# kyshu11027/financial-chatbot-llm

Hardware: AMD Instinct MI355X
Metric: chat turns/sec + p50 TTFT, Llama-3-8B RAG agent at 1/2/4/8 MI355X (higher is better)
Workload: dtype bf16

## Files before the change

financial_chatbot_llm_amd/csrc/kernels/gemm_prefill.hip:

```cpp
#include "common.h"
#include "kv_layout.h"

#include <type_traits>

namespace {

constexpr int TN = 256;
constexpr int TM = 256;
constexpr int BK = 64;
constexpr int HALF = 128 * 128;
constexpr int BUF = 4 * HALF;
constexpr int GM = 4;
enum { H_W0 = 0, H_X0 = 1, H_X1 = 2, H_W1 = 3 };
enum { EPI_BF16 = 0, EPI_SILU = 1, EPI_SLAB = 2, EPI_RESID = 3, EPI_ROPE = 4, EPI_BIAS = 5, EPI_BIAS_GELU = 6,
       EPI_MOE_SILU = 7, EPI_MOE_ROUTE = 8, EPI_SAMPLE = 9, EPI_MOE_SILU_MX = 10, EPI_MOE_ROUTE_MX = 11,
       EPI_LOGPROB = 12, EPI_SAMPLE_LP = 13 };

struct MoeArgs {
  const int* offsets;
  const int* rows;
  const float* xs;
  const float* ws;
  const float* route_w;
  int E;
  unsigned* mxs;
  int nkt;
};

struct SampleArgs {
  const float* temps;
  const unsigned long long* seeds;
  float* pv;
  int* pi;
  int voff, vvalid;
};

struct LogprobArgs {
  const int* targets;
  float* pm;
  float* ps;
  float* pt;
  int* pa;
  int voff, vvalid;
};

struct TailArgs {
  int dpn, L, s;
  float* part;
  int* cnt;
  int gm = 0;
};

struct RopeArgs {
  const int* positions;
  const float* cos_sin;
  const int* slots;
  bf16* q_out;
  bf16* k_cache;
  bf16* v_cache;
  int Hq, Hkv;
  float qscale = 1.f;
};

template <bool FP8>
__device__ __forceinline__ int swz(int r) { return FP8 ? ((r >> 1) & 5) : ((r >> 1) & 7); }

union Frag {
  uint4 u;
  bf16x8 v;
};
typedef int i32x8 __attribute__((ext_vector_type(8)));
union FragPair {
  Frag f[2];
  i32x8 v;
};

__device__ __forceinline__ uint4 pair16(bf16x4 lo, bf16x4 hi) {
  union {
    bf16x4 v;
    uint2 u;
  } a, b;
  a.v = lo;
  b.v = hi;
  const auto x = __builtin_amdgcn_permlane16_swap(a.u.x, b.u.x, false, false);
  const auto y = __builtin_amdgcn_permlane16_swap(a.u.y, b.u.y, false, false);
  return make_uint4(x[0], y[0], x[1], y[1]);
}

template <int N>
__device__ __forceinline__ void wait_vm() {
  asm volatile("s_waitcnt vmcnt(%0)" ::"n"(N) : "memory");
}
__device__ __forceinline__ void wait_lgkm0() { asm volatile("s_waitcnt lgkmcnt(0)" ::: "memory"); }
__device__ __forceinline__ void bar() { __builtin_amdgcn_s_barrier(); }

__device__ __forceinline__ void read_w(const char* __restrict__ h, FragPair (&a)[4], int wa, int rowoff,
                                       const int (&choff)[2]) {
#pragma unroll
  for (int f = 0; f < 4; ++f)
#pragma unroll
    for (int kk = 0; kk < 2; ++kk)
      a[f].f[kk].u = *reinterpret_cast<const uint4*>(h + (wa * 64 + f * 16) * 128 + rowoff + choff[kk]);
}

__device__ __forceinline__ void read_w_tiled(const char* __restrict__ h, FragPair (&a)[4], int wa, int lane) {
#pragma unroll
  for (int f = 0; f < 4; ++f)
#pragma unroll
    for (int kk = 0; kk < 2; ++kk)
      a[f].f[kk].u = *reinterpret_cast<const uint4*>(h + ((wa * 4 + f) * 2 + kk) * 1024 + lane * 16);
}

__device__ __forceinline__ void read_x(const char* __restrict__ h, FragPair (&b)[2], int wb, int rowoff,
                                       const int (&choff)[2]) {
#pragma unroll
  for (int t = 0; t < 2; ++t)
#pragma unroll
    for (int kk = 0; kk < 2; ++kk)
      b[t].f[kk].u = *reinterpret_cast<const uint4*>(h + (wb * 32 + t * 16) * 128 + rowoff + choff[kk]);
}

template <int F0, int T0, bool FP8, bool MXI = false>
__device__ __forceinline__ void mma(f32x4 (&acc)[8][4], const FragPair (&a)[4], const FragPair (&b)[2],
                                    unsigned sc = 0) {
  __builtin_amdgcn_sched_barrier(0);
  __builtin_amdgcn_s_setprio(1);
  if constexpr (FP8 && MXI) {
#pragma unroll
    for (int f = 0; f < 4; ++f) {
      acc[F0 + f][T0] = __builtin_amdgcn_mfma_scale_f32_16x16x128_f8f6f4(a[f].v, b[0].v, acc[F0 + f][T0], 0, 0, 0,
                                                                         127, T0, (int)sc);
      acc[F0 + f][T0 + 1] = __builtin_amdgcn_mfma_scale_f32_16x16x128_f8f6f4(a[f].v, b[1].v, acc[F0 + f][T0 + 1], 0, 0,
                                                                             0, 127, T0 + 1, (int)sc);
    }
#pragma unroll
    for (int f = 0; f < 4; ++f)
#pragma unroll
      for (int t = 0; t < 2; ++t) asm volatile("" : "+v"(acc[F0 + f][T0 + t]));
  } else if constexpr (FP8) {
#pragma unroll
    for (int f = 0; f < 4; ++f)
#pragma unroll
      for (int t = 0; t < 2; ++t)
        acc[F0 + f][T0 + t] = __builtin_amdgcn_mfma_scale_f32_16x16x128_f8f6f4(
            a[f].v, b[t].v, acc[F0 + f][T0 + t], 0, 0, 0, 127, 0, 127);
#pragma unroll
    for (int f = 0; f < 4; ++f)
#pragma unroll
      for (int t = 0; t < 2; ++t) asm volatile("" : "+v"(acc[F0 + f][T0 + t]));
  } else {
#pragma unroll
    for (int kk = 0; kk < 2; ++kk)
#pragma unroll
      for (int f = 0; f < 4; ++f)
#pragma unroll
        for (int t = 0; t < 2; ++t)
          acc[F0 + f][T0 + t] =
              __builtin_amdgcn_mfma_f32_16x16x32_bf16(a[f].f[kk].v, b[t].f[kk].v, acc[F0 + f][T0 + t], 0, 0, 0);
  }
  __builtin_amdgcn_s_setprio(0);
  __builtin_amdgcn_sched_barrier(0);
}

template <int EPI, int ABL = 0, int BAL = 1, bool FP8 = false, bool WT = false>
__global__ void __launch_bounds__(512) gemm_prefill_kernel(const void* __restrict__ Xv, int ldx,
                                                           const void* __restrict__ Wv, int K,
                                                           void* __restrict__ Y, int ldy,
                                                           const bf16* __restrict__ R, int ldr,
                                                           int M, int N, int S, RopeArgs ra, MoeArgs ma,
                                                           SampleArgs sa, TailArgs ta, LogprobArgs la) {
  static_assert(!(WT && FP8), "fragment-tiled W: bf16 only");
  constexpr int ESZ = FP8 ? 1 : 2;
  constexpr int BKE = 128 / ESZ;
  constexpr bool MXI = EPI == EPI_MOE_ROUTE_MX;
  constexpr bool MXO = EPI == EPI_MOE_SILU_MX;
  static_assert(!(MXI || MXO) || (FP8 && BAL), "MX hand-off: fp8 tiles on the balanced schedule");
  constexpr int XL0 = MXI ? 3 : 2;
  const char* __restrict__ X = static_cast<const char*>(Xv);
  const char* __restrict__ W = static_cast<const char*>(Wv);
  __shared__ __attribute__((aligned(1024))) char smem[2 * BUF + (MXI ? 2048 : 0)];
  const int lane = threadIdx.x & 63;
  const int w = __builtin_amdgcn_readfirstlane(threadIdx.x >> 6);
  const int wa = w >> 2, wb = w & 3;
  const int g = lane >> 4, col = lane & 15;

  const int Mt = (M + TM - 1) / TM + (FP8 ? ma.E : 0), Nt = N / TN, tiles = Mt * Nt;
  const bool tail = !FP8 && EPI != EPI_SAMPLE_LP && ta.s > 1 && (int)blockIdx.x >= ta.dpn;
  int s = 0, tile, tu = 0, tj = 0;
  if (tail) {
    const int u = blockIdx.x - ta.dpn;
    tu = u % ta.L;
    tj = u / ta.L;
    tile = ta.dpn + tu;
  } else {
    const int nwg = ta.s > 1 ? ta.dpn : tiles * S;
    int id = blockIdx.x;
    const int xcd = id & 7, q = nwg >> 3, r = nwg & 7;
    id = (xcd < r ? xcd * (q + 1) : r * (q + 1) + (xcd - r) * q) + (id >> 3);
    s = id / tiles;
    tile = id - s * tiles;
  }
  const int GMr = ta.gm > 0 ? ta.gm : GM;
  const int grp = tile / (GMr * Nt), first = grp * GMr, gm = min(Mt - first, GMr);
  const int within = tile - grp * GMr * Nt;
  const int tm = first + within % gm, tn = within / gm;
  int m0 = tm * TM, mend = M, e = 0;
  const int n0 = tn * TN;
  if constexpr (FP8) {
    int rem = tm;
    for (e = 0; e < ma.E; ++e) {
      const int lo = ma.offsets[e], hi = ma.offsets[e + 1], nte = (hi - lo + TM - 1) / TM;
      if (rem < nte) {
        m0 = lo + rem * TM;
        mend = hi;
        break;
      }
      rem -= nte;
    }
    if (e == ma.E) return;
    W += (long)e * N * K;
  }
  int k0, nt;
  if (tail) {
    const int ntot = K / BKE, kb = tj * ntot / ta.s, ke = (tj + 1) * ntot / ta.s;
    k0 = kb * BKE;
    nt = ke - kb;
  } else {
    const int kc = K / S;
    k0 = s * kc;
    nt = kc / BKE;
  }
  PENNY_DASSERT(N % TN == 0 && nt >= 1 && tm < Mt && tn < Nt);

  const char* src[4][2];
  unsigned soff[4][2];
#pragma unroll
  for (int h = 0; h < 4; ++h)
#pragma unroll
    for (int i = 0; i < 2; ++i) {
      const int lr = 16 * w + 8 * i + (lane >> 3);
      const int c = (lane & 7) ^ swz<FP8>(lr);
      if (h == H_W0 || h == H_W1) {
        const int n = n0 + (lr >> 6) * 128 + (h == H_W1 ? 64 : 0) + (lr & 63);
        if constexpr (FP8) soff[h][i] = (unsigned)(((long)n * K + k0) + 16 * c);
        else if constexpr (WT) {
          const int G = n0 / 16 + (w >> 2) * 8 + (w & 3) + (h == H_W1 ? 4 : 0);
          src[h][i] = W + (((long)G * (K / 32) + k0 / 32 + i) * 64 + lane) * 16;
        } else src[h][i] = W + ((long)n * K + k0) * ESZ + 16 * c;
      } else {
        int m = min(m0 + (lr >> 5) * 64 + (h == H_X1 ? 32 : 0) + (lr & 31), mend - 1);
        if (FP8 && ma.rows) m = ma.rows[m];
        if constexpr (FP8) soff[h][i] = (unsigned)(((long)m * ldx + k0) + 16 * c);
        else src[h][i] = X + ((long)m * ldx + k0) * ESZ + 16 * c;
      }
    }
  const unsigned lds0 = (unsigned)(uintptr_t)((__attribute__((address_space(3))) char*)smem);
  const char* mxbase = nullptr;
  if constexpr (MXI) mxbase = reinterpret_cast<const char*>(ma.mxs) + ((long)tm * ma.nkt + k0 / BKE) * 1024 + w * 128;
  auto stage = [&](int h, int t, unsigned buf) {
    if (ABL == 1 && t > 1) return;
#pragma unroll
    for (int i = 0; i < 2; ++i) {
      const unsigned dst = buf + h * HALF + (16 * w + 8 * i) * 128;
      unsigned keep;
      if constexpr (FP8) {
        const unsigned vo = soff[h][i] + (unsigned)t * 128;
        const char* base = (h == H_W0 || h == H_W1) ? W : X;
        asm volatile("s_mov_b32 %0, m0\n\ts_mov_b32 m0, %2\n\ts_nop 0\n\tglobal_load_lds_dwordx4 %1, %3\n\ts_mov_b32 m0, %0"
                     : "=&s"(keep)
                     : "v"(vo), "s"(dst), "s"(base)
                     : "memory");
      } else {
        const char* gp = src[h][i] + (long)t * ((WT && (h == H_W0 || h == H_W1)) ? 2048 : 128);
        asm volatile("s_mov_b32 %0, m0\n\ts_mov_b32 m0, %2\n\ts_nop 0\n\tglobal_load_lds_dwordx4 %1, off\n\ts_mov_b32 m0, %0"
                     : "=&s"(keep)
                     : "v"(gp), "s"(dst)
                     : "memory");
      }
    }
    if constexpr (MXI) {
      if (h == H_X0) {
        const char* gp = mxbase + (long)t * 1024 + lane * 4;
        const unsigned dst = lds0 + 2 * BUF + (t & 1) * 1024 + w * 128;
        unsigned keep;
        if (lane < 32)
          asm volatile("s_mov_b32 %0, m0\n\ts_mov_b32 m0, %2\n\ts_nop 0\n\tglobal_load_lds_dword %1, off\n\ts_mov_b32 m0, %0"
                       : "=&s"(keep)
                       : "v"(gp), "s"(dst)
                       : "memory");
      }
    }
  };
  auto read_sc = [&](int t) -> unsigned {
    if constexpr (MXI)
      return *reinterpret_cast<const unsigned*>(smem + 2 * BUF + (t & 1) * 1024 + wb * 256 + col * 16 + g * 4);
    else
      return 0u;
  };

  const int rowoff = col * 128;
  const int choff[2] = {((FP8 ? 2 * g : g) ^ swz<FP8>(col)) << 4, ((FP8 ? 2 * g + 1 : 4 + g) ^ swz<FP8>(col)) << 4};

  f32x4 acc[8][4];
#pragma unroll
  for (int f = 0; f < 8; ++f)
#pragma unroll
// ... 15 lines not shown
    wait_vm<0>();
  }
  bar();
  if (wa == 1) bar();

  auto phase = [&](auto F0c, auto T0c, const FragPair (&aa)[4], const FragPair (&bb)[2], unsigned sc = 0) {
    constexpr int F0 = decltype(F0c)::value, T0 = decltype(T0c)::value;
    bar();
    wait_lgkm0();
    mma<F0, T0, FP8, MXI>(acc, aa, bb, sc);
    bar();
  };
  using I0 = std::integral_constant<int, 0>;
  using I2 = std::integral_constant<int, 2>;
  using I4 = std::integral_constant<int, 4>;

  if constexpr (BAL) {
    FragPair c0[2];
    unsigned sc = 0;
    auto tile = [&](int t, FragPair (&bc)[2], FragPair (&bn)[2]) {
      const char* cur = smem + (t & 1) * BUF;
      const char* nx = smem + ((t + 1) & 1) * BUF;
      const unsigned lcur = lds0 + (t & 1) * BUF, lnxt = lds0 + ((t + 1) & 1) * BUF;
      const bool more1 = t + 1 < nt, more2 = t + 2 < nt;
      if (ABL != 2 || t == 0) READ_W(cur + H_W0 * HALF);
      sc = read_sc(t);
      if (more1) stage(H_W1, t + 1, lnxt);
      phase(I0{}, I0{}, a, bc, sc);
      if (ABL != 2 || t == 0) read_x(cur + H_X1 * HALF, b1, wb, rowoff, choff);
      if (more2) stage(H_W0, t + 2, lcur);
      phase(I0{}, I2{}, a, b1, sc);
      if (ABL != 2 || t == 0) READ_W(cur + H_W1 * HALF);
      if (more2) {
        stage(H_X0, t + 2, lcur);
        if (ABL != 3) wait_vm<6 + XL0>();
      } else {
        wait_vm<0>();
      }
      phase(I4{}, I2{}, a, b1, sc);
      if (more1 && (ABL != 2 || t == 0)) read_x(nx + H_X0 * HALF, bn, wb, rowoff, choff);
      if (more2) {
        stage(H_X1, t + 2, lcur);
        if (ABL != 3) wait_vm<4 + XL0>();
      } else {
        wait_vm<0>();
      }
      phase(I4{}, I0{}, a, bc, sc);
    };
    read_x(smem + H_X0 * HALF, b0, wb, rowoff, choff);
    int t = 0;
    for (; t + 1 < nt; t += 2) {
      tile(t, b0, c0);
      tile(t + 1, c0, b0);
    }
    if (t < nt) tile(t, b0, c0);
  } else {
    for (int t = 0; t < nt; ++t) {
      const char* cur = smem + (t & 1) * BUF;
      const unsigned lcur = lds0 + (t & 1) * BUF, lnxt = lds0 + ((t + 1) & 1) * BUF;
      const bool more1 = t + 1 < nt, more2 = t + 2 < nt;
      if (ABL != 2 || t == 0) {
        READ_W(cur + H_W0 * HALF);
        read_x(cur + H_X0 * HALF, b0, wb, rowoff, choff);
      }
      if (more1) stage(H_W1, t + 1, lnxt);
      phase(I0{}, I0{}, a, b0);
      if (ABL != 2 || t == 0) read_x(cur + H_X1 * HALF, b1, wb, rowoff, choff);
      if (more2) stage(H_W0, t + 2, lcur);
      phase(I0{}, I2{}, a, b1);
      if (ABL != 2 || t == 0) READ_W(cur + H_W1 * HALF);
      if (more2) stage(H_X0, t + 2, lcur);
      phase(I4{}, I2{}, a, b1);
      if (more2) {
        stage(H_X1, t + 2, lcur);
        if (ABL != 3) wait_vm<6>();
      } else {
        wait_vm<0>();
      }
      phase(I4{}, I0{}, a, b0);
    }
  }
  if (wa == 0) bar();

  if (!FP8 && tail) {
    float* mine = ta.part + ((long)tu * ta.s + tj) * (TM * TN);
#pragma unroll
    for (int f = 0; f < 8; ++f)
#pragma unroll
      for (int t = 0; t < 4; ++t)
        *reinterpret_cast<f32x4*>(mine + ((((w * 8 + f) * 4 + t) * 64 + lane) << 2)) = acc[f][t];
    wait_vm<0>();
    __syncthreads();
    int* flag = reinterpret_cast<int*>(smem);
    if (threadIdx.x == 0) {
      __builtin_amdgcn_fence(__ATOMIC_RELEASE, "agent");
      wait_vm<0>();
      const int old = __hip_atomic_fetch_add(&ta.cnt[tu], 1, __ATOMIC_RELAXED, __HIP_MEMORY_SCOPE_AGENT);
      const int last = old == ta.s - 1;
      if (last) {
        __builtin_amdgcn_fence(__ATOMIC_ACQUIRE, "agent");
        wait_vm<0>();
        __hip_atomic_store(&ta.cnt[tu], 0, __ATOMIC_RELAXED, __HIP_MEMORY_SCOPE_AGENT);
      }
      *reinterpret_cast<volatile int*>(flag) = last;
    }
    __syncthreads();
    if (!*reinterpret_cast<volatile int*>(flag)) return;
    const float* base = ta.part + (long)tu * ta.s * (TM * TN) + ((w * 32 * 64 + lane) << 2);
    for (int j = 0; j < ta.s; ++j) {
      const float* pj = base + (long)j * (TM * TN);
#pragma unroll
      for (int f = 0; f < 8; ++f)
#pragma unroll
        for (int t = 0; t < 4; ++t) {
          const f32x4 v = *reinterpret_cast<const f32x4*>(pj + ((f * 4 + t) * 64 << 2));
          acc[f][t] = j == 0 ? v : acc[f][t] + v;
        }
    }
  }

  const int lane_off = 8 * (g >> 1) + 16 * (g & 1);
  if constexpr (MXO) {
    const float* wsc = ma.ws + (long)e * N + n0 + wa * 128;
    unsigned char* yq = static_cast<unsigned char*>(Y);
    const int ocol = ((n0 + wa * 128) >> 1) + 4 * g;
    unsigned word[2] = {0u, 0u};
#pragma unroll
    for (int t = 0; t < 4; ++t) {
      const int m = m0 + wb * 64 + t * 16 + col;
      const bool valid = m < mend;
      const int mr = min(m, mend - 1);
      const float sx = ma.xs[ma.rows ? ma.rows[mr] : mr];
      float o[4][4];
#pragma unroll
      for (int q = 0; q < 4; ++q) {
        const f32x4 sg = *reinterpret_cast<const f32x4*>(wsc + 32 * q + 4 * g);
        const f32x4 su = *reinterpret_cast<const f32x4*>(wsc + 32 * q + 16 + 4 * g);
#pragma unroll
        for (int r = 0; r < 4; ++r) {
          const float gv = (float)(bf16)(acc[2 * q][t][r] * sx * sg[r]);
          const float uv = (float)(bf16)(acc[2 * q + 1][t][r] * sx * su[r]);
          o[q][r] = (float)(bf16)((float)(bf16)(gv / (1.f + __expf(-gv))) * uv);
        }
      }
#pragma unroll
      for (int bb = 0; bb < 2; ++bb) {
        float amax = 0.f;
#pragma unroll
        for (int q = bb; q < 4; q += 2)
#pragma unroll
          for (int r = 0; r < 4; ++r) amax = fmaxf(amax, fabsf(o[q][r]));
        amax = fmaxf(amax, __shfl_xor(amax, 16, 64));
        amax = fmaxf(amax, __shfl_xor(amax, 32, 64));
        const unsigned bits = __float_as_uint(amax * (1.f / 448.f));
        const int ex = (int)((bits >> 23) & 0xff);
        int X = ex == 0 ? -127 : ex - 127 + ((bits & 0x7fffff) != 0);
        X = max(-127, min(X, 126));
        word[bb] |= (unsigned)(X + 127) << (8 * t);
        const float inv = __uint_as_float((unsigned)(127 - X) << 23);
        if (valid) {
#pragma unroll
          for (int q = bb; q < 4; q += 2) {
            uint32_t pk = 0;
            pk = __builtin_amdgcn_cvt_pk_fp8_f32(o[q][0] * inv, o[q][1] * inv, pk, false);
            pk = __builtin_amdgcn_cvt_pk_fp8_f32(o[q][2] * inv, o[q][3] * inv, pk, true);
            *reinterpret_cast<uint32_t*>(yq + (long)m * ldy + ocol + 16 * q) = pk;
          }
        }
      }
    }
    if (g < 2)
      ma.mxs[((long)tm * ma.nkt + n0 / 256) * 256 + wb * 64 + col * 4 + wa + 2 * g] = g == 0 ? word[0] : word[1];
    return;
  }
#pragma unroll
  for (int t = 0; t < 4; ++t) {
    const int m = m0 + wb * 64 + t * 16 + col;
    if (m >= mend) continue;
    if constexpr (EPI == EPI_MOE_SILU || EPI == EPI_MOE_ROUTE || EPI == EPI_MOE_ROUTE_MX) {
      const float sx = MXI ? 1.f : ma.xs[ma.rows ? ma.rows[m] : m];
      const float* wsc = ma.ws + (long)e * N + n0 + wa * 128;
      if constexpr (EPI == EPI_MOE_SILU) {
        bf16x4 o[4];
#pragma unroll
        for (int q = 0; q < 4; ++q) {
          const f32x4 sg = *reinterpret_cast<const f32x4*>(wsc + 32 * q + 4 * g);
          const f32x4 su = *reinterpret_cast<const f32x4*>(wsc + 32 * q + 16 + 4 * g);
#pragma unroll
          for (int r = 0; r < 4; ++r) {
            const float gv = (float)(bf16)(acc[2 * q][t][r] * sx * sg[r]);
            const float uv = (float)(bf16)(acc[2 * q + 1][t][r] * sx * su[r]);
            o[q][r] = (bf16)((float)(bf16)(gv / (1.f + __expf(-gv))) * uv);
          }
        }
        bf16* y = static_cast<bf16*>(Y) + (long)m * ldy + ((n0 + wa * 128) >> 5) * 16 + lane_off;
#pragma unroll
        for (int q = 0; q < 4; q += 2) *reinterpret_cast<uint4*>(y + 16 * q) = pair16(o[q], o[q + 1]);
      } else {
        const float rw = sx * ma.route_w[m];
        bf16* y = static_cast<bf16*>(Y) + (long)m * ldy + n0 + wa * 128 + lane_off;
// ... 124 lines not shown
      const long blk = slot >= 0 ? slot / KV_BS : 0;
      const int off = slot >= 0 ? slot % KV_BS : 0;
      if (hd < ra.Hq + ra.Hkv) {
        const float* cs = ra.cos_sin + (long)ra.positions[m] * D;
        const float qs = hd < ra.Hq ? ra.qscale : 1.f;
#pragma unroll
        for (int f = 0; f < 4; ++f) {
          const int d = f * 16 + 4 * g;
          const f32x4 co = *reinterpret_cast<const f32x4*>(cs + d), si = *reinterpret_cast<const f32x4*>(cs + 64 + d);
          bf16x4 o1, o2;
#pragma unroll
          for (int r = 0; r < 4; ++r) {
            const float x1 = (float)(bf16)acc[f][t][r], x2 = (float)(bf16)acc[f + 4][t][r];
            o1[r] = (bf16)((x1 * co[r] - x2 * si[r]) * qs);
            o2[r] = (bf16)((x2 * co[r] + x1 * si[r]) * qs);
          }
          if (hd < ra.Hq) {
            bf16* q = ra.q_out + ((long)m * ra.Hq + hd) * D;
            *reinterpret_cast<bf16x4*>(q + d) = o1;
            *reinterpret_cast<bf16x4*>(q + 64 + d) = o2;
          } else {
            bf16* kb = ra.k_cache + (blk * ra.Hkv + (hd - ra.Hq)) * (long)(KV_BS * D);
            *reinterpret_cast<bf16x4*>(kb + k_index(off, d, D)) = o1;
            *reinterpret_cast<bf16x4*>(kb + k_index(off, 64 + d, D)) = o2;
          }
        }
      } else {
        bf16* vb = ra.v_cache + (blk * ra.Hkv + (hd - ra.Hq - ra.Hkv)) * (long)(KV_BS * D);
#pragma unroll
        for (int f = 0; f < 8; ++f)
#pragma unroll
          for (int r = 0; r < 4; ++r) vb[v_index(off, f * 16 + 4 * g + r, D)] = (bf16)acc[f][t][r];
      }
    } else if constexpr (EPI == EPI_SILU) {
      const int col0 = ((n0 + wa * 128) >> 5) * 16;
      bf16x4 o[4];
#pragma unroll
      for (int q = 0; q < 4; ++q)
#pragma unroll
        for (int r = 0; r < 4; ++r) {
          const float gt = (float)(bf16)acc[2 * q][t][r], up = (float)(bf16)acc[2 * q + 1][t][r];
          o[q][r] = (bf16)((float)(bf16)(gt / (1.f + __expf(-gt))) * up);
        }
      bf16* y = static_cast<bf16*>(Y) + (long)m * ldy + col0 + lane_off;
#pragma unroll
      for (int q = 0; q < 4; q += 2) *reinterpret_cast<uint4*>(y + 16 * q) = pair16(o[q], o[q + 1]);
    } else if constexpr (EPI == EPI_SLAB) {
      float* P = static_cast<float*>(Y) + (long)s * M * N + (long)m * N;
#pragma unroll
      for (int f = 0; f < 8; ++f) *reinterpret_cast<f32x4*>(P + n0 + wa * 128 + f * 16 + 4 * g) = acc[f][t];
    } else {
      bf16* y = static_cast<bf16*>(Y) + (long)m * ldy + n0 + wa * 128 + lane_off;
#pragma unroll
      for (int f = 0; f < 8; f += 2) {
        bf16x4 lo, hi;
        if constexpr (EPI == EPI_BIAS || EPI == EPI_BIAS_GELU) {
          const int n = n0 + wa * 128 + f * 16 + 4 * g;
          const bf16x4 b0 = *reinterpret_cast<const bf16x4*>(R + n), b1 = *reinterpret_cast<const bf16x4*>(R + n + 16);
#pragma unroll
          for (int r = 0; r < 4; ++r) {
            float u0 = (float)(bf16)(acc[f][t][r] + (float)b0[r]), u1 = (float)(bf16)(acc[f + 1][t][r] + (float)b1[r]);
            if constexpr (EPI == EPI_BIAS_GELU) {
              u0 = 0.5f * u0 * (1.f + erff(u0 * 0.70710678118654752f));
              u1 = 0.5f * u1 * (1.f + erff(u1 * 0.70710678118654752f));
            }
            lo[r] = (bf16)u0, hi[r] = (bf16)u1;
          }
        } else {
#pragma unroll
          for (int r = 0; r < 4; ++r) lo[r] = (bf16)acc[f][t][r], hi[r] = (bf16)acc[f + 1][t][r];
        }
        Pack8 v;
        v.u = pair16(lo, hi);
        if constexpr (EPI == EPI_RESID) {
          Pack8 rr;
          rr.u = *reinterpret_cast<const uint4*>(R + (long)m * ldr + n0 + wa * 128 + lane_off + 16 * f);
#pragma unroll
          for (int j = 0; j < 8; ++j) v.e[j] = (bf16)((float)v.e[j] + (float)rr.e[j]);
        }
        *reinterpret_cast<uint4*>(y + 16 * f) = v.u;
      }
    }
  }
}

}

#undef READ_W

static int g_group = 0;

template <int EPI, int ABL = 0, int BAL = 1, bool WT = false>
static void launch(dim3 grid, hipStream_t stream, const void* X, int ldx, const void* W, int K, void* Y, int ldy,
                   const void* R, int ldr, int M, int N, int S, const RopeArgs& ra, TailArgs ta = TailArgs{}) {
  ta.gm = g_group;
  hipLaunchKernelGGL((gemm_prefill_kernel<EPI, ABL, BAL, false, WT>), grid, dim3(512), 0, stream, X, ldx, W, K, Y,
                     ldy, (const bf16*)R, ldr, M, N, S, ra, MoeArgs{}, SampleArgs{}, ta, LogprobArgs{});
}

static dim3 grid_for(int M, int N, int S) { return dim3((unsigned)(((M + TM - 1) / TM) * (N / TN) * S)); }

static dim3 tail_plan(int M, int N, int K, int cus, float* ws, long ws_floats, int* cnt, int ncnt, TailArgs& ta) {
  ta = TailArgs{};
  const int T = ((M + TM - 1) / TM) * (N / TN);
  if (cus > 0 && ws && cnt) {
    const int L = T % cus, ntot = K / BK;
    int s = L ? cus / L : 0;
    s = min(s, ntot / 16);
    if (L && s >= 2 && L <= ncnt && (long)L * s * TM * TN <= ws_floats) {
      ta = TailArgs{T - L, L, s, ws, cnt};
      return dim3((unsigned)(T - L + L * s));
    }
  }
  return dim3((unsigned)T);
}

PENNY_API int penny_gemm_prefill_set_group(int gm) {
  if (gm < 0 || gm > 64) return (int)hipErrorInvalidValue;
  g_group = gm;
  return 0;
}

PENNY_API int penny_gemm_prefill(const void* X, int ldx, const void* W, int K, void* Y, int ldy, const void* R,
                                 int ldr, int M, int N, int S, int epi, float* tail_ws, long tail_ws_floats,
                                 int* tail_cnt, int tail_ncnt, int cus, hipStream_t stream) {
  if (M <= 0) return 0;
  if (N % TN || S < 1 || K % (BK * S) || ldx % 8 || epi < 0 || epi > 6 || epi == EPI_ROPE)
    return (int)hipErrorInvalidValue;
  if (epi != EPI_SLAB && (S != 1 || ldy % 8)) return (int)hipErrorInvalidValue;
  if (epi == EPI_RESID && (!R || ldr % 8)) return (int)hipErrorInvalidValue;
  if ((epi == EPI_BIAS || epi == EPI_BIAS_GELU) && !R) return (int)hipErrorInvalidValue;
  if ((long)((M + TM - 1) / TM) * (N / TN) * S > (1L << 30)) return (int)hipErrorInvalidValue;
  TailArgs ta{};
  const dim3 grid = S == 1 ? tail_plan(M, N, K, cus, tail_ws, tail_ws_floats, tail_cnt, tail_ncnt, ta)
                           : grid_for(M, N, S);
  const RopeArgs ra{};
  switch (epi) {
    case EPI_BF16: launch<EPI_BF16>(grid, stream, X, ldx, W, K, Y, ldy, R, ldr, M, N, S, ra, ta); break;
    case EPI_SILU: launch<EPI_SILU>(grid, stream, X, ldx, W, K, Y, ldy, R, ldr, M, N, S, ra, ta); break;
    case EPI_SLAB: launch<EPI_SLAB>(grid, stream, X, ldx, W, K, Y, ldy, R, ldr, M, N, S, ra); break;
    case EPI_BIAS: launch<EPI_BIAS>(grid, stream, X, ldx, W, K, Y, ldy, R, ldr, M, N, S, ra, ta); break;
    case EPI_BIAS_GELU: launch<EPI_BIAS_GELU>(grid, stream, X, ldx, W, K, Y, ldy, R, ldr, M, N, S, ra, ta); break;
    default: launch<EPI_RESID>(grid, stream, X, ldx, W, K, Y, ldy, R, ldr, M, N, S, ra, ta);
  }
  return (int)hipGetLastError();
}

PENNY_API int penny_gemm_prefill_wt(const void* X, int ldx, const void* Wt, int K, void* Y, int ldy, const void* R,
                                    int ldr, int M, int N, int S, int epi, float* tail_ws, long tail_ws_floats,
                                    int* tail_cnt, int tail_ncnt, int cus, hipStream_t stream) {
  if (M <= 0) return 0;
  if (N % TN || S < 1 || K % (BK * S) || ldx % 8 || (epi != EPI_BF16 && epi != EPI_SILU && epi != EPI_SLAB &&
                                                    epi != EPI_RESID))
    return (int)hipErrorInvalidValue;
  if (epi != EPI_SLAB && (S != 1 || ldy % 8)) return (int)hipErrorInvalidValue;
  if (epi == EPI_RESID && (!R || ldr % 8)) return (int)hipErrorInvalidValue;
  TailArgs ta{};
  const dim3 grid = S == 1 ? tail_plan(M, N, K, cus, tail_ws, tail_ws_floats, tail_cnt, tail_ncnt, ta)
                           : grid_for(M, N, S);
  const RopeArgs ra{};
  switch (epi) {
    case EPI_BF16: launch<EPI_BF16, 0, 1, true>(grid, stream, X, ldx, Wt, K, Y, ldy, R, ldr, M, N, S, ra, ta); break;
    case EPI_SILU: launch<EPI_SILU, 0, 1, true>(grid, stream, X, ldx, Wt, K, Y, ldy, R, ldr, M, N, S, ra, ta); break;
    case EPI_SLAB: launch<EPI_SLAB, 0, 1, true>(grid, stream, X, ldx, Wt, K, Y, ldy, R, ldr, M, N, S, ra); break;
    default: launch<EPI_RESID, 0, 1, true>(grid, stream, X, ldx, Wt, K, Y, ldy, R, ldr, M, N, S, ra, ta);
  }
  return (int)hipGetLastError();
}

PENNY_API int penny_gemm_prefill_qkv_rope(const void* X, int ldx, const void* W, int K, int M, const int* positions,
                                          const float* cos_sin, const int* slots, void* q_out, void* k_cache,
                                          void* v_cache, int Hq, int Hkv, float qscale, float* tail_ws,
                                          long tail_ws_floats,
                                          int* tail_cnt, int tail_ncnt, int cus, hipStream_t stream) {
  if (M <= 0) return 0;
  const int N = (Hq + 2 * Hkv) * 128;
  if (Hq <= 0 || Hkv <= 0 || N % TN || K % BK || ldx % 8 || !positions || !cos_sin || !slots || !q_out)
    return (int)hipErrorInvalidValue;
  const RopeArgs ra{positions, cos_sin, slots, (bf16*)q_out, (bf16*)k_cache, (bf16*)v_cache, Hq, Hkv, qscale};
  TailArgs ta{};
  const dim3 grid = tail_plan(M, N, K, cus, tail_ws, tail_ws_floats, tail_cnt, tail_ncnt, ta);
  launch<EPI_ROPE>(grid, stream, X, ldx, W, K, nullptr, 0, nullptr, 0, M, N, 1, ra, ta);
  return (int)hipGetLastError();
}

PENNY_API int penny_gemm_prefill_ablate(const void* X, int ldx, const void* W, int K, void* Y, int ldy, int M, int N,
                                        int ablate, hipStream_t stream) {
  if (M <= 0) return 0;
  if (N % TN || K % BK || ldx % 8 || ldy % 4) return (int)hipErrorInvalidValue;
  const RopeArgs ra{};
  if (ablate == 1) launch<EPI_BF16, 1>(grid_for(M, N, 1), stream, X, ldx, W, K, Y, ldy, nullptr, 0, M, N, 1, ra);
  else if (ablate == 10) launch<EPI_BF16, 0, 0>(grid_for(M, N, 1), stream, X, ldx, W, K, Y, ldy, nullptr, 0, M, N, 1, ra);
  else if (ablate == 3) launch<EPI_BF16, 3>(grid_for(M, N, 1), stream, X, ldx, W, K, Y, ldy, nullptr, 0, M, N, 1, ra);
  else if (ablate == 2) launch<EPI_BF16, 2>(grid_for(M, N, 1), stream, X, ldx, W, K, Y, ldy, nullptr, 0, M, N, 1, ra);
  else launch<EPI_BF16, 0>(grid_for(M, N, 1), stream, X, ldx, W, K, Y, ldy, nullptr, 0, M, N, 1, ra);
  return (int)hipGetLastError();
}

PENNY_API int penny_moe_gemm_prefill_fp8(const void* X, int ldx, const int* rows, const float* xs, const int* offsets,
                                         const void* W, const float* ws, const float* route_w, void* Y, int ldy,
                                         int P, int E, int N, int K, int epi, hipStream_t stream) {
  if (P <= 0) return 0;
  const bool plain = epi >= 16;
// ... 296 lines not shown
```

financial_chatbot_llm_amd/ops/_native.py:

```python
from __future__ import annotations

import ctypes
import os
import threading
from typing import Optional

import torch

_LOCK = threading.Lock()
_LIB: Optional[ctypes.CDLL] = None
_ERR: Optional[str] = None

c_int, c_long, c_float, c_void_p = ctypes.c_int, ctypes.c_long, ctypes.c_float, ctypes.c_void_p
P = c_void_p

_SIGS = {
    "penny_rmsnorm": [P, P, P, P, c_int, c_int, c_float, c_int, P],
    "penny_rmsnorm_slabs": [P, c_int, P, P, P, c_int, c_int, c_float, c_int, P],
    "penny_layernorm": [P, P, P, P, P, c_int, c_int, c_float, c_int, P],
    "penny_silu_mul": [P, P, c_int, c_int, c_int, P],
    "penny_skinny_gemm": [P, c_int, P, c_int, P, c_int, P, c_int, c_int, c_int, c_int, c_int, c_int, P],
    "penny_splitk_gemm": [P, c_int, P, c_int, P, c_int, c_int, c_int, c_int, c_int, P],
    "penny_splitk_reduce": [P, c_int, c_int, c_int, P, c_int, P, c_int, P],
    "penny_splitk_gemm_bf16": [P, c_int, P, c_int, P, c_int, c_int, c_int, c_int, c_int, P],
    "penny_lm_head_stream_sample": [P, c_int, P, c_int, c_int, c_int, c_int, c_int, P, P, P, P, P, c_int, c_int,
                                    c_int, P],
    "penny_lm_sample_final": [P, P, c_int, c_int, P, P, P],
    "penny_gateup_silu_gemm": [P, c_int, P, c_int, P, c_int, c_int, c_int, c_int, c_int, P],
    "penny_gemm_prefill": [P, c_int, P, c_int, P, c_int, P, c_int, c_int, c_int, c_int, c_int,
                           P, c_long, P, c_int, c_int, P],
    "penny_gemm_prefill_wt": [P, c_int, P, c_int, P, c_int, P, c_int, c_int, c_int, c_int, c_int,
                              P, c_long, P, c_int, c_int, P],
    "penny_gemm_prefill_qkv_rope": [P, c_int, P, c_int, c_int, P, P, P, P, P, P, c_int, c_int,
                                    c_float, P, c_long, P, c_int, c_int, P],
    "penny_gemm_mid_variant": [c_int],
    "penny_gemm_mid": [P, c_int, P, c_int, P, c_int, P, c_int, c_int, c_int, c_int, c_int, P],
    "penny_gemm_prefill_ablate": [P, c_int, P, c_int, P, c_int, c_int, c_int, c_int, P],
    "penny_moe_gemm_prefill_fp8": [P, c_int, P, P, P, P, P, P, P, c_int, c_int, c_int, c_int, c_int, c_int, P],
    "penny_probe_mfma_scale": [P, P, P, P, P, c_int, P],
    "penny_moe_gemm_prefill_fp8_mx": [P, c_int, P, P, P, P, P, P, P, c_int, c_int, c_int, c_int, c_int, c_int, P,
                                      c_int, P],
    "penny_gelu": [P, c_long, P],
    "penny_embedding": [P, P, P, c_int, c_int, c_int, c_int, P],
    "penny_rope_qk": [P, P, P, P, c_int, c_int, c_int, c_int, P],
    "penny_rope_kv_write": [P, P, P, P, P, P, P, c_int, c_int, c_int, c_int, c_int, P],
    "penny_rope_kv_write_slabs": [P, c_int, P, P, P, P, P, P, c_int, c_int, c_int, c_int, c_int, P],
    "penny_rope_kv_write_fp8": [P, P, P, P, P, P, P, P, c_int, c_int, c_int, c_int, c_int, P],
    "penny_rope_kv_write_slabs_fp8": [P, c_int, P, P, P, P, P, P, P, c_int, c_int, c_int, c_int, c_int, P],
    "penny_kv_dequant_fp8": [P, P, P, c_long, c_int, c_int, P],
    "penny_attention_decode_fp8": [P, P, P, P, P, P, P, P, P, c_int, c_int, c_int, c_int, c_int, c_int, c_int,
                                   c_float, c_int, P, c_int, c_int, P, P],
    "penny_attention_prefill_fp8": [P, P, P, P, P, P, P, c_int, c_int, c_int, c_int, c_int, c_int, c_float, c_int, P,
                                    P, c_int, P, P],
    "penny_attention_prefill_lean_fp8": [P, P, P, P, P, P, P, c_int, c_int, c_int, c_int, c_float, c_int, P, P,
                                         c_int, P, c_int, P, P, P, P],
    "penny_attention_prefill": [P, P, P, P, P, P, P, c_int, c_int, c_int, c_int, c_int, c_int, c_float, c_int, P, P,
                                c_int, P],
    "penny_attention_prefill_variant": [c_int],
    "penny_gemm_prefill_set_group": [c_int],
    "penny_attention_prefill_lean": [P, P, P, P, P, P, P, c_int, c_int, c_int, c_int, c_float, c_int, P, P, c_int, P,
                                     c_int, P, P, P],
    "penny_splitk_reduce_silu": [P, c_int, c_int, c_int, P, c_int, P],
    "penny_attention_decode": [P, P, P, P, P, P, P, P, P, c_int, c_int, c_int, c_int, c_int, c_int, c_int, c_int,
                               c_float, c_int, P, c_int, c_int, P],
    "penny_sample": [P, c_int, c_long, P, P, P, P, P, P, c_int, c_int, P],
    "penny_sample_fsm": [P, c_int, c_long, P, P, P, P, P, P, c_int, c_int, P, P, P, c_int, c_int, P, P, P, c_int, P,
                         c_int, P],
    "penny_fsm_build_masks": [P, P, P, P, P, c_int, c_int, c_int, c_int, c_int, c_int, P],
    "penny_pen_reset": [P, c_int, c_int, c_int, c_int, P, c_int, P],
    "penny_pen_add": [P, c_int, c_int, c_int, P, c_int, P],
    "penny_pen_apply": [P, c_int, c_long, P, P, P, P, P, P, c_int, c_int, P, c_int, c_int, P],
    "penny_lora_shrink": [P, c_long, P, P, c_int, c_int, c_int, P, c_int, c_int, P],
    "penny_lora_expand": [P, c_int, P, P, P, P, c_int, P, c_int, c_int, P, c_int, c_long, c_int, c_int, P],
    "penny_kv_gather_blocks": [P, c_long, c_long, c_int, c_int, P, c_int, P, P],
    "penny_kv_scatter_blocks": [P, c_long, c_long, c_int, c_int, P, c_int, P, P],
    "penny_lm_head_sample": [P, c_int, P, c_int, c_int, c_int, P, P, P, P, P],
    "penny_lm_head_sample_shard": [P, c_int, P, c_int, c_int, c_int, c_int, c_int, P, P, P, P, P],
    "penny_lm_head_logprob": [P, c_int, P, c_int, c_int, c_int, c_int, c_int, P, P, P, P, P],
    "penny_lm_head_sample_logprob": [P, c_int, P, c_int, c_int, c_int, c_int, c_int, P, P, P, P, P, P],
    "penny_lm_head_stream_sample_logprob": [P, c_int, P, c_int, c_int, c_int, c_int, c_int, P, P, P, P, P, c_int,
                                            c_int, c_int, P],
    "penny_lm_sample_logprob_final": [P, P, P, P, P, c_int, c_int, P, P, P],
    "penny_token_logprob": [P, c_int, c_long, P, P, c_int, c_int, P],
    "penny_topn_logprob": [P, c_int, c_long, P, P, c_int, P, P, P, c_int, c_int, P],
    "penny_sample_shard": [P, c_int, c_long, P, P, P, P, c_int, c_int, c_int, P],
    "penny_topk_topp_threshold": [P, c_int, c_long, P, P, P, P, c_int, c_int, P],
    "penny_moe_route": [P, c_int, c_int, c_int, P, P, P, P, P],
    "penny_moe_route_quant": [P, c_int, P, c_int, c_int, c_int, c_int, P, P, P, P, P, P, P, P, P],
    "penny_quant_rows_fp8": [P, c_int, c_int, c_int, P, P, P],
    "penny_silu_quant_rows_fp8": [P, c_int, c_int, P, P, P],
    "penny_moe_gemm_fp8": [P, P, P, P, P, P, P, P, c_int, c_int, c_int, c_int, c_int, P],
    "penny_moe_combine": [P, P, c_int, c_int, c_int, P, P],
    "penny_moe_combine_weighted": [P, P, P, c_int, c_int, c_int, P, P],
    "penny_filtered_topk": [P, P, P, c_long, c_int, P, P, P, P, c_int, c_int, P, P, P, c_int, P, P, P, P],
    "penny_filtered_topk_hybrid": [P, P, P, c_long, c_int, P, P, P, P, P, P, P, P, P, c_int, c_int, P, P, P, c_int,
                                   P, P, P, P],
    "penny_lex_df_add": [P, c_long, P, P],
}


def lib_path() -> str:
    if os.environ.get("PENNY_KERNEL_LIB"):
        return os.environ["PENNY_KERNEL_LIB"]
    from .._build import kernel_lib
    return kernel_lib(os.environ.get("PENNY_KERNEL_DEBUG") == "1")


def load(build_if_missing: bool = True) -> ctypes.CDLL:
    global _LIB, _ERR
    if _LIB is not None:
        return _LIB
    with _LOCK:
        if _LIB is not None:
            return _LIB
        path = lib_path()
        if not os.path.exists(path) and build_if_missing:
            from .._build import build_kernels
            build_kernels(debug=os.environ.get("PENNY_KERNEL_DEBUG") == "1")
        try:
            lib = ctypes.CDLL(path, mode=ctypes.RTLD_GLOBAL)
        except OSError as e:
            _ERR = str(e)
            raise RuntimeError(f"penny kernel library unavailable: {e}") from e
        for name, args in _SIGS.items():
            fn = getattr(lib, name)
            fn.argtypes = args
            fn.restype = c_int
        _LIB = lib
        return lib


def available() -> bool:
    try:
        load(build_if_missing=False)
        return True
    except Exception:
        return False


_FORCE_TORCH_OPS = os.environ.get("PENNY_FORCE_TORCH_OPS") == "1"


# ... 23 lines not shown
```

financial_chatbot_llm_amd/ops/gemm.py:

```python
from __future__ import annotations

import os
from typing import Dict, List, Optional, Tuple, Union

import torch
import torch.nn.functional as F

from . import _native as N
from .activation import silu_mul

EPI = {None: 0, "silu": 1, "residual": 2}
MAX_SKINNY_M = 64
TUNING: Dict[Tuple[int, int], Tuple[int, int]] = {(6144, 4096): (2, 4), (4096, 4096): (1, 4)}
SKINNY_MAX_M: Dict[Tuple[int, int], int] = {(6144, 4096): 16, (4096, 4096): 32}


def _config(N_: int, K: int, epilogue: Optional[str]) -> Tuple[int, int]:
    if (N_, K) in TUNING:
        return TUNING[(N_, K)]
    ntf = 2
    wgs = N_ // (16 * ntf)
    nw = 8 if wgs < 512 else 4
    if K % (nw * 128):
        nw = 4 if K % 512 == 0 else 1
# ... 417 lines not shown
        return y
    if slabs and residual is None:
        return Slabs(P)
    return splitk_reduce(P, residual=residual)


def qkv_rope_fused(x: torch.Tensor, w: torch.Tensor, D: int, k_cache: Optional[torch.Tensor] = None) -> bool:
    if k_cache is not None and k_cache.dtype == torch.float8_e4m3fn:
        return False
    M, K = x.shape
    N_ = w.shape[0]
    if D != 128 or M <= 256 or not prefill_ok(x, w):
        return False
    mode = os.environ.get("PENNY_PREFILL_GEMM", "1")
    if mode == "0":
        return False
    if mode == "force":
        return True
    rows = PREFILL_POLICY.get((N_, K))
    if rows is None:
        return _default_choice(M, N_, K, None) == "hip"
    return next(c for max_m, c in rows if M <= max_m) == "fused"


def prefill_ok(x: torch.Tensor, w: torch.Tensor) -> bool:
    M, K = x.shape
    N_ = w.shape[0]
    return (N.use_native(x) and os.environ.get("PENNY_PREFILL_GEMM", "1") != "0" and N_ % 256 == 0
            and K % 64 == 0 and x.stride(1) == 1 and x.stride(0) % 8 == 0 and w.is_contiguous())


def prefill_gemm(x: torch.Tensor, w: torch.Tensor, epilogue: Optional[str] = None, S: int = 1,
                 residual: Optional[torch.Tensor] = None, out: Optional[torch.Tensor] = None,
                 bias: Optional[torch.Tensor] = None) -> torch.Tensor:
    M, K = x.shape
    N_ = w.shape[0]
    if not N.use_native(x):
        if epilogue == "slabs":
            xs = x.float().view(M, S, K // S).transpose(0, 1)
            return torch.einsum("smk,snk->smn", xs, w.float().view(N_, S, K // S).transpose(0, 1))
        y = F.linear(x.float(), w.float(), bias.float() if bias is not None else None).to(x.dtype)
        if epilogue == "bias_gelu":
            y = F.gelu(y.float()).to(x.dtype)
        elif epilogue == "silu":
            y = silu_mul(y, interleave16=True)
        elif epilogue == "residual":
            y = (y.float() + residual.float()).to(x.dtype)
        return out.copy_(y) if out is not None else y
    if epilogue == "slabs":
        y = out if out is not None else torch.empty((S, M, N_), dtype=torch.float32, device=x.device)
        ldy = N_
    else:
        S = 1
        cols = N_ // 2 if epilogue == "silu" else N_
        y = out if out is not None else torch.empty((M, cols), dtype=x.dtype, device=x.device)
        ldy = y.stride(0)
    R = bias if epilogue in ("bias", "bias_gelu") else residual
    N.call("penny_gemm_prefill", N.ptr(x), x.stride(0), N.ptr(w), K, N.ptr(y), ldy, N.ptr(R),
           residual.stride(0) if residual is not None else 0, M, N_, S, PREFILL_EPI[epilogue],
           *tail_workspace(x.device), N.stream())
    return y


def prefill_gemm_tiled(x: torch.Tensor, wt: torch.Tensor, N_: int, epilogue: Optional[str] = None, S: int = 1,
                       residual: Optional[torch.Tensor] = None, out: Optional[torch.Tensor] = None) -> torch.Tensor:
    M, K = x.shape
    if not N.use_native(x):
        return prefill_gemm(x, untile_weight(wt), epilogue, S, residual=residual, out=out)
    if epilogue == "slabs":
        y = out if out is not None else torch.empty((S, M, N_), dtype=torch.float32, device=x.device)
        ldy = N_
    else:
        S = 1
        cols = N_ // 2 if epilogue == "silu" else N_
        y = out if out is not None else torch.empty((M, cols), dtype=x.dtype, device=x.device)
        ldy = y.stride(0)
    N.call("penny_gemm_prefill_wt", N.ptr(x), x.stride(0), N.ptr(wt), K, N.ptr(y), ldy, N.ptr(residual),
           residual.stride(0) if residual is not None else 0, M, N_, S, PREFILL_EPI[epilogue],
           *tail_workspace(x.device), N.stream())
    return y


_TAIL_WS: Dict[Tuple[int, int], Tuple[torch.Tensor, torch.Tensor, int]] = {}


def tail_workspace(dev: torch.device) -> Tuple:
    if os.environ.get("PENNY_GEMM_TAIL", "1") == "0":
        return (None, 0, None, 0, 0)
    key = (dev.index if dev.index is not None else torch.cuda.current_device(), torch.cuda.current_stream(dev).cuda_stream)
    ent = _TAIL_WS.get(key)
    if ent is None:
        cus = torch.cuda.get_device_properties(dev).multi_processor_count
        part = torch.empty((cus * 256 * 256,), dtype=torch.float32, device=dev)
        cnt = torch.zeros((cus,), dtype=torch.int32, device=dev)
        ent = _TAIL_WS[key] = (part, cnt, cus)
    part, cnt, cus = ent
    return (N.ptr(part), part.numel(), N.ptr(cnt), cnt.numel(), cus)


BGE_TILE_MAX_M = 2048


def linear_bias(x: torch.Tensor, w: torch.Tensor, b: torch.Tensor, gelu: bool = False) -> torch.Tensor:
    M, K = x.shape
    N_ = w.shape[0]
    mode = os.environ.get("PENNY_PREFILL_GEMM", "1")
    if mode != "0" and prefill_ok(x, w) and (M <= BGE_TILE_MAX_M or mode == "force" or
                                            prefill_choice(M, N_, K, "bias_gelu" if gelu else "bias") == "hip"):
        return prefill_gemm(x, w, "bias_gelu" if gelu else "bias", bias=b)
    y = F.linear(x, w, b)
    if gelu:
        from .activation import gelu_
        return gelu_(y)
    return y


def prefill_qkv_rope(x: torch.Tensor, w: torch.Tensor, positions: torch.Tensor, cos_sin: torch.Tensor,
                     slots: torch.Tensor, k_cache: torch.Tensor, v_cache: torch.Tensor, Hq: int,
                     Hkv: int, qscale: float = 1.0) -> torch.Tensor:
    from .attention import rope_kv_write
    M, K = x.shape
    if not N.use_native(x):
        if qscale == 1.0:
            return rope_kv_write(F.linear(x.float(), w.float()).to(x.dtype), positions, cos_sin, slots, k_cache,
                                 v_cache, Hq, Hkv, 128)
        from .attention import _rope_ref
        qkv = F.linear(x.float(), w.float()).to(x.dtype)
        rope_kv_write(qkv, positions, cos_sin, slots, k_cache, v_cache, Hq, Hkv, 128)
        qr = _rope_ref(qkv[:, :Hq * 128].float().view(M, Hq, 128), positions, cos_sin)
        return (qr * qscale).to(x.dtype)
    q = torch.empty((M, Hq, 128), dtype=x.dtype, device=x.device)
    N.call("penny_gemm_prefill_qkv_rope", N.ptr(x), x.stride(0), N.ptr(w), K, M, N.ptr(positions), N.ptr(cos_sin),
           N.ptr(slots), N.ptr(q), N.ptr(k_cache), N.ptr(v_cache), Hq, Hkv, float(qscale), *tail_workspace(x.device),
           N.stream())
    return q


def untile_weight(wt: torch.Tensor) -> torch.Tensor:
    G, KS = wt.shape[0], wt.shape[1]
    return wt.view(G, KS, 4, 16, 8).permute(0, 3, 1, 2, 4).reshape(G * 16, KS * 32)
```

Before: 42.35.

## Add stream-K tail scheduling for prefill GEMM wave-quantization tail

Adds a stream-K mode for the leftover tiles of the last wave in the prefill GEMM. Each of the CU-count work units now walks a contiguous range of K-iterations that may span two tiles, instead of splitting every tail tile into equal K slices. A host-side cost model picks stream-K or the old equal split, and the fp32 partial workspace is doubled so each unit can hold two partials. This aims to balance the final wave across CUs, at the cost of more partial-sum traffic, atomic fixup logic and a kernel template variant that loops over segments with goto.

```diff
diff --git a/financial_chatbot_llm_amd/csrc/kernels/gemm_prefill.hip b/financial_chatbot_llm_amd/csrc/kernels/gemm_prefill.hip
--- a/financial_chatbot_llm_amd/csrc/kernels/gemm_prefill.hip
+++ b/financial_chatbot_llm_amd/csrc/kernels/gemm_prefill.hip
@@ -49,7 +49,26 @@
   float* part;
   int* cnt;
   int gm = 0;
+  int sk = 0;
+  int minseg = 1;
 };
+
+__host__ __device__ inline int sk_bound(int u, int units, int L, int nt, int minseg) {
+  int b = (int)((unsigned)u * (unsigned)(L * nt) / (unsigned)units);
+  const int r = b % nt;
+  if (r < minseg) b -= r;
+  else if (nt - r < minseg) b += nt - r;
+  return b;
+}
+
+__host__ __device__ inline int sk_touch(int j, int u, int units, int L, int nt, int minseg, int& ua, int& ub) {
+  ua = ub = u;
+  while (ua > 0 && sk_bound(ua, units, L, nt, minseg) > j * nt) --ua;
+  while (ub + 1 < units && sk_bound(ub + 1, units, L, nt, minseg) < (j + 1) * nt) ++ub;
+  int n = 0;
+  for (int v = ua; v <= ub; ++v) n += sk_bound(v + 1, units, L, nt, minseg) > sk_bound(v, units, L, nt, minseg);
+  return n;
+}
 
 struct RopeArgs {
   const int* positions;
@@ -162,7 +181,7 @@
   __builtin_amdgcn_sched_barrier(0);
 }
 
-template <int EPI, int ABL = 0, int BAL = 1, bool FP8 = false, bool WT = false>
+template <int EPI, int ABL = 0, int BAL = 1, bool FP8 = false, bool WT = false, bool SK = false>
 __global__ void __launch_bounds__(512) gemm_prefill_kernel(const void* __restrict__ Xv, int ldx,
                                                            const void* __restrict__ Wv, int K,
                                                            void* __restrict__ Y, int ldy,
@@ -170,6 +189,7 @@
                                                            int M, int N, int S, RopeArgs ra, MoeArgs ma,
                                                            SampleArgs sa, TailArgs ta, LogprobArgs la) {
   static_assert(!(WT && FP8), "fragment-tiled W: bf16 only");
+  static_assert(!SK || (!FP8 && EPI != EPI_SAMPLE_LP && EPI != EPI_SLAB), "stream-K tail: bf16 tail epilogues");
   constexpr int ESZ = FP8 ? 1 : 2;
   constexpr int BKE = 128 / ESZ;
   constexpr bool MXI = EPI == EPI_MOE_ROUTE_MX;
@@ -185,15 +205,44 @@
   const int g = lane >> 4, col = lane & 15;
 
   const int Mt = (M + TM - 1) / TM + (FP8 ? ma.E : 0), Nt = N / TN, tiles = Mt * Nt;
-  const bool tail = !FP8 && EPI != EPI_SAMPLE_LP && ta.s > 1 && (int)blockIdx.x >= ta.dpn;
+  const bool tail = !FP8 && EPI != EPI_SAMPLE_LP && (SK ? ta.sk > 0 : ta.s > 1) &&
+                    (int)blockIdx.x >= ta.dpn;
+  int seg = 0, nseg = 1, unit = 0, ukb = 0, uke = 0;
+  if constexpr (SK) {
+    if (tail) {
+      const int i = blockIdx.x - ta.dpn;
+      unit = (ta.sk & 7) ? i : (i & 7) * (ta.sk >> 3) + (i >> 3);
+      ukb = sk_bound(unit, ta.sk, ta.L, K / BKE, ta.minseg);
+      uke = sk_bound(unit + 1, ta.sk, ta.L, K / BKE, ta.minseg);
+      if (uke == ukb) return;
+      nseg = (uke - 1) / (K / BKE) - ukb / (K / BKE) + 1;
+    }
+  }
+#define NEXT_SEGMENT()                                                         \
+  do {                                                                         \
+    if constexpr (SK) {                                                        \
+      if (++seg < nseg) {                                                      \
+        __syncthreads();  \
+        goto next_segment;                                                     \
+      }                                                                        \
+    }                                                                          \
+  } while (0)
+next_segment:
   int s = 0, tile, tu = 0, tj = 0;
-  if (tail) {
+  int klo = 0, khi = 0;
+  if (SK && tail) {
+    const int ntot = K / BKE;
+    tu = ukb / ntot + seg;
+    tile = ta.dpn + tu;
+    klo = max(ukb, tu * ntot) - tu * ntot;
+    khi = min(uke, (tu + 1) * ntot) - tu * ntot;
+  } else if (tail) {
     const int u = blockIdx.x - ta.dpn;
     tu = u % ta.L;
     tj = u / ta.L;
     tile = ta.dpn + tu;
   } else {
-    const int nwg = ta.s > 1 ? ta.dpn : tiles * S;
+    const int nwg = (SK ? ta.sk > 0 : ta.s > 1) ? ta.dpn : tiles * S;
     int id = blockIdx.x;
     const int xcd = id & 7, q = nwg >> 3, r = nwg & 7;
     id = (xcd < r ? xcd * (q + 1) : r * (q + 1) + (xcd - r) * q) + (id >> 3);
@@ -221,7 +270,10 @@
     W += (long)e * N * K;
   }
   int k0, nt;
-  if (tail) {
+  if (SK && tail) {
+    k0 = klo * BKE;
+    nt = khi - klo;
+  } else if (tail) {
     const int ntot = K / BKE, kb = tj * ntot / ta.s, ke = (tj + 1) * ntot / ta.s;
     k0 = kb * BKE;
     nt = ke - kb;
@@ -403,8 +455,10 @@
   }
   if (wa == 0) bar();
 
-  if (!FP8 && tail) {
-    float* mine = ta.part + ((long)tu * ta.s + tj) * (TM * TN);
+  if (!FP8 && tail && !(SK && nt == K / BKE)) {
+    float* mine = ta.part + (SK ? (long)unit * 2 + seg : (long)tu * ta.s + tj) * (TM * TN);
+    int ua = 0, ub = 0, target = ta.s;
+    if constexpr (SK) target = sk_touch(tu, unit, ta.sk, ta.L, K / BKE, ta.minseg, ua, ub);
 #pragma unroll
     for (int f = 0; f < 8; ++f)
 #pragma unroll
@@ -417,7 +471,7 @@
       __builtin_amdgcn_fence(__ATOMIC_RELEASE, "agent");
       wait_vm<0>();
       const int old = __hip_atomic_fetch_add(&ta.cnt[tu], 1, __ATOMIC_RELAXED, __HIP_MEMORY_SCOPE_AGENT);
-      const int last = old == ta.s - 1;
+      const int last = old == target - 1;
       if (last) {
         __builtin_amdgcn_fence(__ATOMIC_ACQUIRE, "agent");
         wait_vm<0>();
@@ -426,17 +480,37 @@
       *reinterpret_cast<volatile int*>(flag) = last;
     }
     __syncthreads();
-    if (!*reinterpret_cast<volatile int*>(flag)) return;
-    const float* base = ta.part + (long)tu * ta.s * (TM * TN) + ((w * 32 * 64 + lane) << 2);
-    for (int j = 0; j < ta.s; ++j) {
-      const float* pj = base + (long)j * (TM * TN);
-#pragma unroll
-      for (int f = 0; f < 8; ++f)
-#pragma unroll
-        for (int t = 0; t < 4; ++t) {
-          const f32x4 v = *reinterpret_cast<const f32x4*>(pj + ((f * 4 + t) * 64 << 2));
-          acc[f][t] = j == 0 ? v : acc[f][t] + v;
-        }
+    if (!*reinterpret_cast<volatile int*>(flag)) {
+      NEXT_SEGMENT();
+      return;
+    }
+    if constexpr (SK) {
+      bool first = true;
+      for (int u = ua; u <= ub; ++u) {
+        const int b0 = sk_bound(u, ta.sk, ta.L, K / BKE, ta.minseg);
+        if (sk_bound(u + 1, ta.sk, ta.L, K / BKE, ta.minseg) == b0) continue;
+        const float* pj = ta.part + ((long)u * 2 + (b0 < tu * (K / BKE))) * (TM * TN) + ((w * 32 * 64 + lane) << 2);
+#pragma unroll
+        for (int f = 0; f < 8; ++f)
+#pragma unroll
+          for (int t = 0; t < 4; ++t) {
+            const f32x4 v = *reinterpret_cast<const f32x4*>(pj + ((f * 4 + t) * 64 << 2));
+            acc[f][t] = first ? v : acc[f][t] + v;
+          }
+        first = false;
+      }
+    } else {
+      const float* base = ta.part + (long)tu * ta.s * (TM * TN) + ((w * 32 * 64 + lane) << 2);
+      for (int j = 0; j < ta.s; ++j) {
+        const float* pj = base + (long)j * (TM * TN);
+#pragma unroll
+        for (int f = 0; f < 8; ++f)
+#pragma unroll
+          for (int t = 0; t < 4; ++t) {
+            const f32x4 v = *reinterpret_cast<const f32x4*>(pj + ((f * 4 + t) * 64 << 2));
+            acc[f][t] = j == 0 ? v : acc[f][t] + v;
+          }
+      }
     }
   }
 
@@ -727,11 +801,13 @@
       }
     }
   }
+  NEXT_SEGMENT();
 }
 
 }
 
 #undef READ_W
+#undef NEXT_SEGMENT
 
 static int g_group = 0;
 
@@ -739,19 +815,75 @@
 static void launch(dim3 grid, hipStream_t stream, const void* X, int ldx, const void* W, int K, void* Y, int ldy,
                    const void* R, int ldr, int M, int N, int S, const RopeArgs& ra, TailArgs ta = TailArgs{}) {
   ta.gm = g_group;
+  if constexpr (EPI != EPI_SLAB && ABL == 0 && BAL == 1) {
+    if (ta.sk > 0) {
+      hipLaunchKernelGGL((gemm_prefill_kernel<EPI, ABL, BAL, false, WT, true>), grid, dim3(512), 0, stream, X, ldx, W,
+                         K, Y, ldy, (const bf16*)R, ldr, M, N, S, ra, MoeArgs{}, SampleArgs{}, ta, LogprobArgs{});
+      return;
+    }
+  }
   hipLaunchKernelGGL((gemm_prefill_kernel<EPI, ABL, BAL, false, WT>), grid, dim3(512), 0, stream, X, ldx, W, K, Y,
                      ldy, (const bf16*)R, ldr, M, N, S, ra, MoeArgs{}, SampleArgs{}, ta, LogprobArgs{});
 }
 
 static dim3 grid_for(int M, int N, int S) { return dim3((unsigned)(((M + TM - 1) / TM) * (N / TN) * S)); }
+
+constexpr int SK_MINSEG = 8;
+constexpr float SK_KT = 2.2f, SK_PRO = 4.f, SK_PART = 0.14f;
+
+enum { TAIL_OLD = 0, TAIL_SK = 1, TAIL_AUTO = 2 };
+static int g_tail_mode = TAIL_AUTO, g_tail_cus = 0;
+
+static int equal_split(int L, int ntot, int cus) {
+  const int s = L ? cus / L : 0;
+  return min(s, ntot / 16);
+}
+
+static float equal_split_cost(int L, int ntot, int s) {
+  return s >= 2 ? (float)((ntot + s - 1) / s) + SK_PART * L * s : (float)ntot;
+}
+
+static bool sk_plan(int L, int ntot, int cus, bool forced, int& minseg, float& cost) {
+  if (L <= 0 || L >= cus || (long)L * ntot * (cus + 1) >= (1L << 31)) return false;
+  const int U = L * ntot / cus;
+  if (!forced && U < SK_MINSEG) return false;
+  minseg = max(1, min(min(SK_MINSEG, U), ntot / 4));
+  float walk = 0.f;
+  int parts = 0;
+  for (int u = 0; u < cus; ++u) {
+    const int b0 = sk_bound(u, cus, L, ntot, minseg), b1 = sk_bound(u + 1, cus, L, ntot, minseg);
+    if (b1 == b0) continue;
+    const int segs = (b1 - 1) / ntot - b0 / ntot + 1;
+    walk = fmaxf(walk, (float)(b1 - b0) + SK_PRO * (segs - 1));
+    parts += segs - (b1 - b0 == ntot && b0 % ntot == 0);
+  }
+  cost = SK_KT * walk + SK_PART * parts;
+  return true;
+}
 
 static dim3 tail_plan(int M, int N, int K, int cus, float* ws, long ws_floats, int* cnt, int ncnt, TailArgs& ta) {
   ta = TailArgs{};
   const int T = ((M + TM - 1) / TM) * (N / TN);
   if (cus > 0 && ws && cnt) {
+    if (g_tail_cus > 0) cus = g_tail_cus;
     const int L = T % cus, ntot = K / BK;
-    int s = L ? cus / L : 0;
-    s = min(s, ntot / 16);
+    const int s = equal_split(L, ntot, cus);
+    thread_local struct { int L, ntot, cus, mode, ok, minseg; } memo = {0, 0, 0, -1, 0, 1};
+    if (g_tail_mode != TAIL_OLD && L && L <= ncnt && 2L * cus * TM * TN <= ws_floats) {
+      if (memo.L != L || memo.ntot != ntot || memo.cus != cus || memo.mode != g_tail_mode) {
+        float cost = 0.f;
+        int minseg = 1;
+        bool ok = sk_plan(L, ntot, cus, g_tail_mode == TAIL_SK, minseg, cost);
+        if (ok && g_tail_mode == TAIL_AUTO) ok = cost < equal_split_cost(L, ntot, s);
+        memo = {L, ntot, cus, g_tail_mode, ok, minseg};
+      }
+      if (memo.ok) {
+        ta = TailArgs{T - L, L, 0, ws, cnt};
+        ta.sk = cus;
+        ta.minseg = memo.minseg;
+        return dim3((unsigned)(T - L + cus));
+      }
+    }
     if (L && s >= 2 && L <= ncnt && (long)L * s * TM * TN <= ws_floats) {
       ta = TailArgs{T - L, L, s, ws, cnt};
       return dim3((unsigned)(T - L + L * s));
@@ -764,6 +896,37 @@
   if (gm < 0 || gm > 64) return (int)hipErrorInvalidValue;
   g_group = gm;
   return 0;
+}
+
+PENNY_API int penny_gemm_prefill_set_tail(int mode, int cus) {
+  if (mode < TAIL_OLD || mode > TAIL_AUTO || cus < 0 || cus > 1024) return (int)hipErrorInvalidValue;
+  g_tail_mode = mode;
+  g_tail_cus = cus;
+  return 0;
+}
+
+PENNY_API int penny_gemm_prefill_tail_plan(int T, int nt, int cus, int mode, int* out, int cap) {
+  if (T <= 0 || nt <= 0 || cus <= 0 || mode < TAIL_OLD || mode > TAIL_AUTO || cap < 5) return -1;
+  const int L = T % cus, s = equal_split(L, nt, cus);
+  int minseg = 1;
+  float cost = 0.f;
+  bool sk = mode != TAIL_OLD && sk_plan(L, nt, cus, mode == TAIL_SK, minseg, cost);
+  if (sk && mode == TAIL_AUTO) sk = cost < equal_split_cost(L, nt, s);
+  const bool split = !sk && L && s >= 2;
+  out[0] = sk ? 2 : split ? 1 : 0;
+  out[1] = sk || split ? T - L : T;
+  out[2] = sk || split ? L : 0;
+  out[3] = sk ? cus : split ? s : 1;
+  out[4] = sk ? minseg : 0;
+  if (!sk) return 5;
+  if (cap < 5 + cus + 1 + L) return -1;
+  for (int u = 0; u <= cus; ++u) out[5 + u] = sk_bound(u, cus, L, nt, minseg);
+  for (int j = 0, u = 0; j < L; ++j) {
+    while (out[5 + u + 1] <= j * nt) ++u;
+    int ua, ub;
+    out[5 + cus + 1 + j] = sk_touch(j, u, cus, L, nt, minseg, ua, ub);
+  }
+  return 5 + cus + 1 + L;
 }
 
 PENNY_API int penny_gemm_prefill(const void* X, int ldx, const void* W, int K, void* Y, int ldy, const void* R,
diff --git a/financial_chatbot_llm_amd/ops/_native.py b/financial_chatbot_llm_amd/ops/_native.py
--- a/financial_chatbot_llm_amd/ops/_native.py
+++ b/financial_chatbot_llm_amd/ops/_native.py
@@ -58,6 +58,8 @@
                                 c_int, P],
     "penny_attention_prefill_variant": [c_int],
     "penny_gemm_prefill_set_group": [c_int],
+    "penny_gemm_prefill_set_tail": [c_int, c_int],
+    "penny_gemm_prefill_tail_plan": [c_int, c_int, c_int, c_int, P, c_int],
     "penny_attention_prefill_lean": [P, P, P, P, P, P, P, c_int, c_int, c_int, c_int, c_float, c_int, P, P, c_int, P,
                                      c_int, P, P, P],
     "penny_splitk_reduce_silu": [P, c_int, c_int, c_int, P, c_int, P],
diff --git a/financial_chatbot_llm_amd/ops/gemm.py b/financial_chatbot_llm_amd/ops/gemm.py
--- a/financial_chatbot_llm_amd/ops/gemm.py
+++ b/financial_chatbot_llm_amd/ops/gemm.py
@@ -523,6 +523,26 @@
 
 
 _TAIL_WS: Dict[Tuple[int, int], Tuple[torch.Tensor, torch.Tensor, int]] = {}
+TAIL_MODES = {"old": 0, "streamk": 1, "auto": 2}
+
+
+def set_tail_mode(mode: str = "auto", cus: int = 0) -> None:
+    N.call("penny_gemm_prefill_set_tail", TAIL_MODES[mode], cus)
+
+
+def tail_plan(T: int, nt: int, cus: int, mode: str = "auto") -> Dict:
+    import ctypes
+    cap = 5 + cus + 1 + T % cus
+    out = (ctypes.c_int * cap)()
+    n = N.load().penny_gemm_prefill_tail_plan(T, nt, cus, TAIL_MODES[mode], out, cap)
+    if n < 5:
+        raise ValueError(f"no tail plan for T={T} nt={nt} cus={cus}")
+    plan = {"kind": ("whole", "split", "streamk")[out[0]], "dpn": out[1], "L": out[2]}
+    if out[0] == 2:
+        plan.update(units=out[3], minseg=out[4], bounds=list(out[5:5 + cus + 1]), targets=list(out[5 + cus + 1:n]))
+    else:
+        plan["s"] = out[3]
+    return plan
 
 
 def tail_workspace(dev: torch.device) -> Tuple:
@@ -532,7 +552,7 @@
     ent = _TAIL_WS.get(key)
     if ent is None:
         cus = torch.cuda.get_device_properties(dev).multi_processor_count
-        part = torch.empty((cus * 256 * 256,), dtype=torch.float32, device=dev)
+        part = torch.empty((2 * cus * 256 * 256,), dtype=torch.float32, device=dev)
         cnt = torch.zeros((cus,), dtype=torch.int32, device=dev)
         ent = _TAIL_WS[key] = (part, cnt, cus)
     part, cnt, cus = ent
```

Result: no change. 42.25 (median of 2 runs) (-0.2%).
